# kpreid/all-is-cubes

Measured on NVIDIA H100. Metric: Mrays/s, higher is better.
Workload: dtype f64 geometry / f32 colour

## Files before the change

### all-is-cubes_b200/csrc/aicb200.cu

```cuda
#include <algorithm>
#include <array>
#include <cmath>
#include <cstdio>
#include <cstdlib>
#include <cstring>
#include <initializer_list>
#include <mutex>
#include <string>
#include <unordered_map>
#include <vector>

#include <cuda_runtime.h>

#include "brick_room.h"
#include "internal.h"

using namespace aicb;

static thread_local std::string g_last_error = "";

aicb_status aicb_fail(aicb_status st, const std::string &msg) {
    g_last_error = msg;
    return st;
}
// ... 117 lines not shown
    const uint32_t pal = pal_off + pal_base;
    float palf;
    std::memcpy(&palf, &pal, 4);
    return make_float4(e.x, e.y, palf, 0.0f);
}

static aicb_status flatten_block(const aicb_block_desc &b, BlockRec &r, uint8_t &kind, std::vector<uint16_t> &bricks,
                                 std::vector<float4> &palette, std::vector<float2> &pal_tab) {
    std::memset(&r, 0, sizeof r);
    const uint32_t res = b.resolution;
    if (res == 0 || (res & (res - 1)) || res > 128) return fail(AICB_ERR_INVALID, "block resolution must be 1..128, power of 2");
    auto push_voxel = [&](const aicb_voxel &v) {
        palette.push_back(make_float4(v.rgba[0], v.rgba[1], v.rgba[2], v.rgba[3]));
        palette.push_back(make_float4(v.emission[0], v.emission[1], v.emission[2], 0.0f));
        pal_tab.push_back(surface_entry(v.rgba[3]));
    };
    bool single = false;
    aicb_voxel sv = AIR_VOXEL;
    if (b.indices == nullptr) {
        single = true;
        if (b.n_palette) {
            if (!b.palette) return fail(AICB_ERR_INVALID, "palette is NULL");
            sv = b.palette[0];
        }
    } else {
        const uint64_t nvox = (uint64_t)b.voxel_bounds.size[0] * b.voxel_bounds.size[1] * b.voxel_bounds.size[2];
        if (nvox != b.n_indices) return fail(AICB_ERR_INVALID, "n_indices does not match voxel_bounds");
        for (int a = 0; a < 3; a++) {
            int64_t lo = b.voxel_bounds.lower[a], hi = lo + (int64_t)b.voxel_bounds.size[a];
            if (lo < 0 || hi > (int64_t)res) return fail(AICB_ERR_INVALID, "voxel_bounds must lie within [0, resolution)^3");
        }
        if (!b.palette && b.n_palette) return fail(AICB_ERR_INVALID, "palette is NULL");
        for (size_t k = 0; k < b.n_indices; k++)
            if (b.indices[k] >= b.n_palette) return fail(AICB_ERR_INVALID, "voxel index out of palette range");
        if (res == 1) {
            single = true;
            sv = (nvox == 1 && b.voxel_bounds.lower[0] == 0 && b.voxel_bounds.lower[1] == 0 && b.voxel_bounds.lower[2] == 0)
                     ? b.palette[b.indices[0]]
                     : AIR_VOXEL;
        }
    }
    if (b.is_air) {
        kind = KIND_INVISIBLE;
        r.kind_res = KIND_INVISIBLE | (1u << 8);
    } else if (single) {
        kind = voxel_invisible(sv) ? KIND_INVISIBLE : KIND_SINGLE;
        r.kind_res = kind | (1u << 8);
        r.pal_off = (uint32_t)(palette.size() / 2);
        r.vsize[0] = r.vsize[1] = r.vsize[2] = 1;
        push_voxel(sv);
    } else {
        if (b.n_palette > 32768) return fail(AICB_ERR_UNSUPPORTED, "block palettes above 32768 entries are not supported");
        kind = KIND_RECURSIVE;
        r.kind_res = KIND_RECURSIVE | (res << 8);
        for (int a = 0; a < 3; a++) {
            r.vlo[a] = (int16_t)b.voxel_bounds.lower[a];
            r.vsize[a] = (uint16_t)b.voxel_bounds.size[a];
        }
        if (bricks.size() + b.n_indices > 0xffffffffull) return fail(AICB_ERR_INVALID, "brick pool exceeds 2^32 voxels");
        r.brick_off = (uint32_t)bricks.size();
        r.pal_off = (uint32_t)(palette.size() / 2);
        for (size_t k = 0; k < b.n_indices; k++) {
            uint16_t v = b.indices[k];
            bricks.push_back((uint16_t)(v | (voxel_invisible(b.palette[v]) ? 0x8000u : 0u)));
        }
        for (size_t k = 0; k < b.n_palette; k++) push_voxel(b.palette[k]);
    }
    return AICB_OK;
}

typedef void (*kernel_fn)(const TraceParams, uint32_t);

template <bool V, bool W, bool AUX>
static kernel_fn kernel_of() {
    return trace_kernel<V, W, AUX>;
}

static kernel_fn select_kernel(bool volumetric, bool wide, bool aux) {
#define PICK(V, W, A) if (volumetric == V && wide == W && aux == A) return kernel_of<V, W, A>();
    PICK(false, false, false) PICK(false, false, true) PICK(false, true, false) PICK(false, true, true)
    PICK(true, false, false) PICK(true, false, true) PICK(true, true, false) PICK(true, true, true)
#undef PICK
    return nullptr;
}

template <typename... KArgs, typename... Args>
static cudaError_t launch_after(bool overlap, void (*kern)(KArgs...), unsigned grid, unsigned block, cudaStream_t st, Args... args) {
    cudaLaunchConfig_t cfg;
    std::memset(&cfg, 0, sizeof cfg);
    cfg.gridDim = dim3(grid, 1, 1);
    cfg.blockDim = dim3(block, 1, 1);
    cfg.dynamicSmemBytes = 0;
    cfg.stream = st;
    cudaLaunchAttribute attr[1];
    attr[0].id = cudaLaunchAttributeProgrammaticStreamSerialization;
    attr[0].val.programmaticStreamSerializationAllowed = 1;
    cfg.attrs = attr;
    cfg.numAttrs = overlap ? 1 : 0;
    return cudaLaunchKernelEx(&cfg, kern, args...);
}

struct CubeDelta {
    uint32_t idx, cell, light, has_light;
};

static __global__ void scatter_cubes_kernel(const CubeDelta *ops, uint32_t n, uint32_t wide, void *cells, uint32_t *light) {
    const uint32_t i = blockIdx.x * blockDim.x + threadIdx.x;
    if (i >= n) return;
    const CubeDelta op = ops[i];
    if (wide) ((uint32_t *)cells)[op.idx] = op.cell; else ((uint16_t *)cells)[op.idx] = (uint16_t)op.cell;
    if (op.has_light) light[op.idx] = op.light;
}

static __device__ __forceinline__ uint32_t widened_cell(uint32_t w) { return (w & 0x3fffu) | ((w >> 14) << 16); }

static __global__ void __launch_bounds__(256) widen_cells_kernel(const uint16_t *__restrict__ in, uint32_t *__restrict__ out,
                                                                 size_t n) {
    const size_t stride = (size_t)gridDim.x * blockDim.x, first = (size_t)blockIdx.x * blockDim.x + threadIdx.x;
    const size_t n8 = n / 8;
    for (size_t i = first; i < n8; i += stride) {
        const uint4 v = __ldcs(reinterpret_cast<const uint4 *>(in) + i);
        __stcs(reinterpret_cast<uint4 *>(out) + 2 * i,
               make_uint4(widened_cell(v.x & 0xffffu), widened_cell(v.x >> 16), widened_cell(v.y & 0xffffu),
                          widened_cell(v.y >> 16)));
        __stcs(reinterpret_cast<uint4 *>(out) + 2 * i + 1,
               make_uint4(widened_cell(v.z & 0xffffu), widened_cell(v.z >> 16), widened_cell(v.w & 0xffffu),
                          widened_cell(v.w >> 16)));
    }
    for (size_t i = n8 * 8 + first; i < n; i += stride) out[i] = widened_cell(in[i]);
}

static __global__ void __launch_bounds__(256) fill_cells_kernel(uint16_t *__restrict__ cells, size_t n, uint32_t word) {
    const size_t stride = (size_t)gridDim.x * blockDim.x, first = (size_t)blockIdx.x * blockDim.x + threadIdx.x;
    const uint32_t pair = word | word << 16;
    const size_t n8 = n / 8;
    for (size_t i = first; i < n8; i += stride) __stcs(reinterpret_cast<uint4 *>(cells) + i, make_uint4(pair, pair, pair, pair));
    for (size_t i = n8 * 8 + first; i < n; i += stride) cells[i] = (uint16_t)word;
}

struct PoolSegment {
    uint64_t src, dst, bytes;
};

static __global__ void __launch_bounds__(256) compact_pool_kernel(const uint8_t *__restrict__ src, uint8_t *__restrict__ dst,
                                                                  const PoolSegment *__restrict__ segs, uint32_t n_segs) {
    for (uint32_t k = blockIdx.x; k < n_segs; k += gridDim.x) {
        const PoolSegment g = segs[k];
        const uint64_t shift = g.src - g.dst;
        const uint64_t c0 = (g.dst + 15) / 16, c1 = (g.dst + g.bytes) / 16;
        const uint32_t s = (uint32_t)(shift & 15), b = (s & 3) * 8;
        for (uint64_t c = c0 + threadIdx.x; c < c1; c += blockDim.x) {
            const uint4 *p = reinterpret_cast<const uint4 *>(src + ((c * 16 + shift) & ~15ull));
            const uint4 lo = p[0];
            uint4 out = lo;
            if (s) {
                const uint4 hi = p[1];
                const uint32_t w[8] = {lo.x, lo.y, lo.z, lo.w, hi.x, hi.y, hi.z, hi.w};
#define FS(i) __funnelshift_r(w[i], w[(i) + 1], b)
                switch (s >> 2) {
                    case 0: out = make_uint4(FS(0), FS(1), FS(2), FS(3)); break;
                    case 1: out = make_uint4(FS(1), FS(2), FS(3), FS(4)); break;
                    case 2: out = make_uint4(FS(2), FS(3), FS(4), FS(5)); break;
                    default: out = make_uint4(FS(3), FS(4), FS(5), FS(6)); break;
                }
#undef FS
            }
// ... 120 lines not shown
    P.task_counter = ctx->d_tile_counter;
    P.refill_threshold = REFILL_THRESHOLD;
    P.tail_divisor = TAIL_DIVISOR;
    P.event_threshold = EVENT_THRESHOLD;

    sc->pending = true;
    sc->pending_pixels = pixels;
    sc->pending_rays = pixels * (P.antialias ? 4 : 1);
    sc->pending_out_bytes_per_pixel =
        P.target.out_srgb8 ? 4 : (tgt == TGT_TEX ? 12 : (tgt == TGT_TERM ? 24 : (P.target.out_rgba16f ? 8 : 16)));

    P.n_samples = P.antialias ? 4 : 1;
    const bool fused = (opt->lighting_display == AICB_LIGHT_NONE || opt->lighting_display == AICB_LIGHT_FLAT) &&
                       !ctx->deep_frames;
    const uint64_t total_tasks = (uint64_t)P.n_tasks * P.n_samples;
    uint64_t CHUNK = (uint64_t)4 << 20;
    {
        const uint64_t per_task = sizeof(RayRecordA) + sizeof(RayRecordB) + sizeof(TaskOut) + 4 * N_BINS +
                                  (uint64_t)ctx->hits_per_task * (sizeof(HitRecord) + (fused ? 0 : sizeof(ShadedHit)));
        uint64_t fit = ((uint64_t)8 << 30) / per_task;
        if (fit < (1u << 17)) fit = 1u << 17;
        if (fit < CHUNK) CHUNK = fit & ~(uint64_t)127;
    }
    const uint64_t chunk_cap = total_tasks < CHUNK ? total_tasks : CHUNK;
    uint64_t cap = chunk_cap * ctx->hits_per_task;
    if (cap < (1u << 16)) cap = 1u << 16;
    if (cap > 0xfffffff0ull) cap = 0xfffffff0ull;
    cap &= ~(uint64_t)(HIT_CHUNK - 1);
    P.hit_capacity = (uint32_t)cap;
    TRY(ctx->primary.size(chunk_cap, P.hit_capacity, !fused));
    ctx->primary.bind(P, chunk_cap, !fused);
    P.ray_counter = ctx->d_tile_counter + 2;
    sc->pending_fused = fused;
    P.hit_counter = ctx->d_tile_counter + 1;
    P.bin_count = ctx->d_tile_counter + 4;
    P.bin_stride = (uint32_t)chunk_cap;
    P.overflow_flag = (unsigned int *)(P.counters + 7);
    if (stream != ctx->stream.get()) CU(cudaStreamWaitEvent(stream, ctx->ev_delta.get(), 0));
    if (ctx->frame_in_flight && ctx->last_stream != stream) CU(cudaStreamWaitEvent(stream, ctx->ev1.get(), 0));
    ctx->frame_in_flight = true;
    ctx->last_stream = stream;
    ctx->last_scene = sc;
    CU(cudaMemsetAsync(P.counters, 0, 8 * sizeof(unsigned long long) + 2 * (4 + N_BINS) * sizeof(unsigned int), stream));
    CU(cudaEventRecord(ctx->ev0.get(), stream));
    if (total_tasks > 0) {
        const bool volumetric = opt->transparency == AICB_TRANSPARENCY_VOLUMETRIC;
        const int lc = opt->lighting_display == AICB_LIGHT_NONE ? LC_NONE
                       : (opt->lighting_display == AICB_LIGHT_FLAT ? LC_FLAT
                          : (opt->lighting_display == AICB_LIGHT_BOUNCE ? LC_BOUNCE : LC_INTERP));
        TraceParams Q;
        const bool bounce = lc == LC_BOUNCE;
        if (bounce) {
            TRY(ctx->secondary.size(chunk_cap, P.hit_capacity, true));
            TRY(ctx->d_bounce.ensure(chunk_cap * 104 + 256));
            char *b = ctx->d_bounce.get<char>();
            P.bounce_mode = BOUNCE_PRIMARY;
            P.bounce_samples = opt->bounce_samples;
            P.bounce_rays = (double *)b;
            P.bounce_rng = (unsigned long long *)(b + chunk_cap * 48);
            P.bounce_sum = (float4 *)(b + chunk_cap * 80);
            P.bounce_req = (uint32_t *)(b + chunk_cap * 96);
            P.ray_index = (uint32_t *)(b + chunk_cap * 100);
            Q = P;
            Q.ray_index = nullptr;
            Q.bounce_mode = BOUNCE_SECONDARY;
            Q.rays = P.bounce_rays;
            Q.tiles_y = 1;
            Q.shard_count = 1; Q.shard_index = 0; Q.strip_rows = 1;
            Q.antialias = 0;
            Q.n_samples = 1;
            Q.task_base = 0;
            Q.lighting = AICB_LIGHT_FLAT;
            Q.include_sky = 1;
            Q.exposure = 1.0f;
            Q.out_full_frame = 0;
            Q.target = {};
            ctx->secondary.bind(Q, chunk_cap, true);
            Q.task_counter = ctx->d_tile_counter + (4 + N_BINS);
            Q.hit_counter = Q.task_counter + 1;
            Q.ray_counter = Q.task_counter + 2;
            Q.bin_count = Q.task_counter + 4;
            Q.debug_warp_times = nullptr;
        }
        kernel_fn k = select_kernel(volumetric, sc->ds.wide_cells != 0, out.aux);
        int blocks_per_sm = 0;
        CU(cudaOccupancyMaxActiveBlocksPerMultiprocessor(&blocks_per_sm, k, WARPS_PER_BLOCK * 32, 0));
        if (blocks_per_sm < 1) blocks_per_sm = 1;
        for (uint64_t base = 0; base < total_tasks; base += CHUNK) {
            const uint32_t n = (uint32_t)(total_tasks - base < CHUNK ? total_tasks - base : CHUNK);
            P.task_base = (uint32_t)base;
            const bool first = base == 0;
            if (!first) CU(cudaMemsetAsync(ctx->d_tile_counter, 0, (4 + N_BINS) * sizeof(unsigned int), stream));
            const bool prof = ctx->profile_kernels && first;
            const bool stage = first && ctx->stage_timing;
            if (stage) cudaEventRecord(ctx->ev_k[0].get(), stream);
            gen_kernel<<<(n + 127) / 128, 128, 0, stream>>>(P, n);
            if (stage) cudaEventRecord(ctx->ev_k[1].get(), stream);
            uint64_t want = ((uint64_t)n + WARPS_PER_BLOCK * 32 - 1) / (WARPS_PER_BLOCK * 32);
            uint64_t grid = (uint64_t)ctx->num_sms * blocks_per_sm;
            if (grid > want) grid = want;
            if (prof) {
                TRY(ctx->d_debug.ensure(4 * 8 * (size_t)ctx->num_sms * 64 * WARPS_PER_BLOCK));
                P.debug_warp_times = ctx->d_debug.get<unsigned long long>();
                ctx->debug_warps = (uint32_t)grid * WARPS_PER_BLOCK;
            }
            const bool overlap = !stage && !prof && !bounce;
            CU(launch_after(overlap, k, (unsigned)grid, WARPS_PER_BLOCK * 32, stream, P, n));
            P.debug_warp_times = nullptr;
            if (stage) cudaEventRecord(ctx->ev_k[2].get(), stream);
            if (fused) {
                const unsigned rb = (n + 127) / 128;
                CU(launch_after(overlap, resolve_for(lc, tgt), rb, 128, stream, P, n));
                if (stage) cudaEventRecord(ctx->ev_k[3].get(), stream);
            } else if (!bounce) {
                switch (lc) {
                    case LC_NONE: CU(launch_after(overlap, shade_kernel<LC_NONE>, ctx->num_sms * SHADE_BLOCKS_PER_SM, 128, stream, P)); break;
                    case LC_FLAT: CU(launch_after(overlap, shade_kernel<LC_FLAT>, ctx->num_sms * SHADE_BLOCKS_PER_SM, 128, stream, P)); break;
                    default: CU(launch_after(overlap, shade_kernel<LC_INTERP>, ctx->num_sms * SHADE_BLOCKS_PER_SM, 128, stream, P)); break;
                }
                if (stage) cudaEventRecord(ctx->ev_k[3].get(), stream);
                const uint32_t n_pixels = n / P.n_samples;
                CU(launch_after(overlap, encode_for(tgt), (n_pixels + 127) / 128, 128, stream, P, n));
                if (stage) cudaEventRecord(ctx->ev_k[4].get(), stream);
            } else {
                shade_kernel<LC_BOUNCE><<<ctx->num_sms * SHADE_BLOCKS_PER_SM, 128, 0, stream>>>(P);
                const unsigned tb = (n + 127) / 128;
                bounce_select_kernel<<<tb, 128, 0, stream>>>(P, n);
                Q.n_rays = n;
                Q.n_tasks = n;
                Q.tiles_x = (n + 31) / 32;
                for (uint32_t pass = 0; pass < P.bounce_samples; pass++) {
                    Q.bounce_pass = pass;
                    CU(cudaMemsetAsync(Q.task_counter, 0, (4 + N_BINS) * sizeof(unsigned int), stream));
                    bounce_gen_kernel<<<tb, 128, 0, stream>>>(P, n);
                    gen_kernel<<<tb, 128, 0, stream>>>(Q, n);
                    k<<<(unsigned)grid, WARPS_PER_BLOCK * 32, 0, stream>>>(Q, n);
                    shade_kernel<LC_FLAT><<<ctx->num_sms * SHADE_BLOCKS_PER_SM, 128, 0, stream>>>(Q);
                    encode_kernel<TGT_FRAME><<<tb, 128, 0, stream>>>(Q, n);
                }
                bounce_resolve_kernel<<<tb, 128, 0, stream>>>(P, n);
                if (stage) cudaEventRecord(ctx->ev_k[3].get(), stream);
                const uint32_t n_pixels = n / P.n_samples;
                encode_for(tgt)<<<(n_pixels + 127) / 128, 128, 0, stream>>>(P, n);
                if (stage) cudaEventRecord(ctx->ev_k[4].get(), stream);
            }
        }
        CU(cudaGetLastError());
    }
    CU(cudaEventRecord(ctx->ev1.get(), stream));
    return AICB_OK;
}

static aicb_status finish(aicb_scene *sc, aicb_render_info *info) {
    aicb_ctx *ctx = sc->ctx;
    if (ctx->last_scene != sc)
        return fail(AICB_ERR_BUSY, "the context's last frame belongs to another scene (one frame per context is tracked)");
    CU(cudaEventSynchronize(ctx->ev1.get()));
    ctx->frame_in_flight = false;
    unsigned long long c[8];
    CU(cudaMemcpy(c, ctx->d_counters.get(), sizeof c, cudaMemcpyDeviceToHost));
    sc->pending = false;
    if (ctx->profile_kernels && sc->pending_rays) {
        float t[4] = {0, 0, 0, 0};
        for (int i = 0; i < (sc->pending_fused ? 3 : 4); i++) cudaEventElapsedTime(&t[i], ctx->ev_k[i].get(), ctx->ev_k[i + 1].get());
        if (ctx->d_debug && ctx->debug_warps) {
            std::vector<unsigned long long> w(4 * (size_t)ctx->debug_warps);
            cudaMemcpy(w.data(), ctx->d_debug.get(), w.size() * 8, cudaMemcpyDeviceToHost);
            unsigned long long t0 = ~0ull, t1 = 0, passes = 0, rays = 0;
            for (uint32_t i = 0; i < ctx->debug_warps; i++) { t0 = std::min(t0, w[4 * i]); t1 = std::max(t1, w[4 * i + 1]); passes += w[4 * i + 2]; rays += w[4 * i + 3]; }
            std::vector<double> ends;
// ... 1279 lines not shown
```

### all-is-cubes_b200/csrc/internal.h

```cpp
#pragma once
#include <memory>
#include <mutex>
#include <string>
#include <utility>
#include <vector>

#include <cuda_runtime.h>

#include "trace_kernel.cuh"

aicb_status aicb_fail(aicb_status st, const std::string &msg);
aicb_status aicb_cuda_fail(cudaError_t e, const char *what);
#define CU(call)                                                   \
    do {                                                           \
        cudaError_t e__ = (call);                                  \
        if (e__ != cudaSuccess) return aicb_cuda_fail(e__, #call); \
    } while (0)
#define TRY(call)                                  \
    do {                                           \
        aicb_status st__ = (call);                 \
        if (st__ != AICB_OK) return st__;          \
    } while (0)

struct DeviceMemory {
// ... 55 lines not shown
};
using DeviceBuffer = Buffer<DeviceMemory>;
using PinnedBuffer = Buffer<PinnedMemory>;

struct EventDestroy {
    void operator()(cudaEvent_t e) const { cudaEventDestroy(e); }
};
struct StreamDestroy {
    void operator()(cudaStream_t s) const { cudaStreamDestroy(s); }
};
using Event = std::unique_ptr<CUevent_st, EventDestroy>;
using Stream = std::unique_ptr<CUstream_st, StreamDestroy>;

inline aicb_status create_event(Event &e, unsigned int flags) {
    cudaEvent_t raw = nullptr;
    CU(cudaEventCreateWithFlags(&raw, flags));
    e.reset(raw);
    return AICB_OK;
}

inline uint32_t cell_word(uint32_t id, uint8_t kind, bool wide) { return id | ((uint32_t)kind << (wide ? 16 : 14)); }

struct ChunkStreams {
    DeviceBuffer rays, task_out, hits, shaded, bin_list;

    aicb_status size(uint64_t chunk_cap, uint32_t hit_capacity, bool shade) {
        TRY(rays.ensure(chunk_cap * (sizeof(aicb::RayRecordA) + sizeof(aicb::RayRecordB)) + 16));
        TRY(task_out.ensure(chunk_cap * sizeof(aicb::TaskOut) + 16));
        TRY(hits.ensure((size_t)hit_capacity * sizeof(aicb::HitRecord) + 64));
        if (shade) TRY(shaded.ensure((size_t)hit_capacity * sizeof(aicb::ShadedHit) + 64));
        return bin_list.ensure((size_t)aicb::N_BINS * chunk_cap * 4 + 64);
    }
    void bind(aicb::TraceParams &P, uint64_t chunk_cap, bool shade) const {
        P.rays_a = rays.get<aicb::RayRecordA>();
        P.rays_b = (aicb::RayRecordB *)(rays.get<char>() + chunk_cap * sizeof(aicb::RayRecordA));
        P.task_out = task_out.get<aicb::TaskOut>();
        P.hits = hits.get<aicb::HitRecord>();
        P.shaded = shade ? shaded.get<aicb::ShadedHit>() : nullptr;
        P.bin_list = bin_list.get<uint32_t>();
    }
    void release_hits() {
        hits.reset();
        shaded.reset();
    }
};

struct LightChart {
    DeviceBuffer pre, chains, node_rel, euler, term_scratch;
    uint32_t nodes = 0, n_chains = 0, n_euler = 0, walk_blocks = 0;
};

struct LightState {
    struct Own {
        DeviceBuffer sky_term;
        DeviceBuffer overflow;
        DeviceBuffer overflow_count;
    } own;
    struct Shared {
        DeviceBuffer pending;
        DeviceBuffer tile_max;
        DeviceBuffer list, new_light, diff;
        DeviceBuffer counters;
        DeviceBuffer changes;
        DeviceBuffer dirty, push_targets;
    } shared;

    aicb_status ensure(aicb_scene *s, size_t replica, size_t n_replicas, const std::vector<float4> *terms);

    uint32_t *changed() const { return own.overflow.get<uint32_t>(); }
    uint32_t *chunk_sums() const { return shared.diff.get<uint32_t>(); }
    uint32_t *taken_indices() const { return shared.list.get<uint32_t>(); }
    uint32_t *taken_texels() const { return shared.new_light.get<uint32_t>(); }
};

struct aicb_ctx {
    int device = 0;
    int num_sms = 0;
    Stream stream;
    Event ev0, ev1;
    Event ev_light[2];
    Event ev_join;
    Event ev_k[5];
    bool profile_kernels = false;
    bool stage_timing = true;
    PinnedBuffer h_delta;
    DeviceBuffer d_delta;
    Event ev_delta;
    DeviceBuffer d_debug;
    uint32_t debug_warps = 0;
    DeviceBuffer d_counters;
    unsigned int *d_tile_counter = nullptr;
    DeviceBuffer d_lut;
    DeviceBuffer d_out, d_aux;
    ChunkStreams primary, secondary;
    DeviceBuffer d_bounce;
    uint32_t hits_per_task = 8;
    uint32_t shallow_frames = 0;
    bool deep_frames = false;
    PinnedBuffer h_stage;
    bool frame_in_flight = false;
    cudaStream_t last_stream = nullptr;
    struct aicb_scene *last_scene = nullptr;
    DeviceBuffer d_task_aux;
    DeviceBuffer d_task_depth;
    DeviceBuffer d_task_text;
    LightChart light_chart;
    std::mutex mu;
};

struct BlockTable {
    struct Extent {
        uint32_t brick_off, n_bricks;
        uint32_t pal_off, n_pal;
    };

    DeviceBuffer blocks;
    DeviceBuffer blk_tab;
    DeviceBuffer light;
    DeviceBuffer bricks;
    DeviceBuffer palette;
    DeviceBuffer pal_tab;
    std::vector<uint8_t> kind;
    std::vector<uint32_t> light_flags;
    std::vector<Extent> extent;
    size_t n_bricks = 0, n_palette = 0;
    size_t dead_bricks = 0, dead_pal = 0;

    size_t block_count() const { return kind.size(); }
    size_t bytes() const {
        return block_count() * (sizeof(aicb::BlockRec) + sizeof(float4) + sizeof(LightBlockDev)) + n_bricks * 2 +
               n_palette * sizeof(float4) + n_palette / 2 * sizeof(float2);
    }
    void bind(aicb::DeviceScene &ds) const {
        ds.blocks = blocks.get<aicb::BlockRec>();
        ds.blk_tab = blk_tab.get<float4>();
        ds.bricks = bricks.get<uint16_t>();
        ds.palette = palette.get<float4>();
        ds.pal_tab = pal_tab.get<float2>();
    }
};

struct aicb_scene {
    aicb_ctx *ctx = nullptr;
    aicb::DeviceScene ds{};
    size_t volume = 0;
    uint64_t device_bytes = 0;
    DeviceBuffer d_cells;
    DeviceBuffer d_light;
    BlockTable blocks;
    bool pending = false;
    uint64_t pending_rays = 0;
    uint64_t pending_pixels = 0;
    uint32_t pending_out_bytes_per_pixel = 0;
    bool pending_fused = false;
    std::vector<uint16_t> h_ids;
    LightState light;
    uint32_t light_max_distance = 0;
    uint64_t light_stats[4] = {0, 0, 0, 0};
};

struct Outputs {
    aicb::TargetParams target{};
    int kind = aicb::TGT_FRAME;
    bool full_frame = false;
    bool aux = false;
    const double *rays = nullptr;
// ... 88 lines not shown
```

### all-is-cubes_b200/csrc/trace_kernel.cuh

```cuda
#pragma once
#include <cstdint>
#include <type_traits>
#include <cuda_runtime.h>

#include "../../include/aicb200.h"

#ifdef __CUDACC__
#include <cuda_fp16.h>
#endif

struct LightBlockDev {
    float face_color[7][4];
    float emission[3];
    uint32_t flags;
};
static_assert(sizeof(LightBlockDev) == 128, "LightBlockDev must be 128 bytes");

namespace aicb {

constexpr uint32_t KIND_SINGLE = 0;
constexpr uint32_t KIND_RECURSIVE = 1;
constexpr uint32_t KIND_INVISIBLE = 2;

struct BlockRec {
// ... 710 lines not shown
        lv.base = 0;
        Caster c;
        c.tmx = c.tmy = c.tmz = c.last_t = 0.0;
        c.rx = c.ry = c.rz = 0;
        c.face = 0;
        c.idx = 0;
        bool valid;
        running = caster_begin(c, r, o[0], o[1], o[2], lv, &valid);
        rec.ox = r.ox; rec.oy = r.oy; rec.oz = r.oz; rec.dx = r.dx; rec.dy = r.dy; rec.dz = r.dz;
        rb.tdx = r.tdx; rb.tdy = r.tdy; rb.tdz = r.tdz;
        rb.half_over_len = r.half_over_len;
        rb.tmx = c.tmx; rb.tmy = c.tmy; rb.tmz = c.tmz; rb.last_t = c.last_t;
        rb.rx = c.rx; rb.ry = c.ry; rb.rz = c.rz;
        rb.task = i;
        rec.flags = ((uint32_t)c.face & 7u) | (running ? 8u : 0u) | (valid ? 16u : 0u) | 32u | ((uint32_t)(r.sx + 1) << 6) |
                    ((uint32_t)(r.sy + 1) << 8) | ((uint32_t)(r.sz + 1) << 10) | (octant << 12);
        if (running) {
            const float lo3[3] = {(float)lv.lox, (float)lv.loy, (float)lv.loz};
            const float n3[3] = {(float)lv.nx, (float)lv.ny, (float)lv.nz};
            float tn = 0.0f, tf = 3.0e38f, l1 = 0.0f;
#pragma unroll
            for (int a = 0; a < 3; a++) {
                const float da = (float)d[a], oa = (float)o[a];
                if (da != 0.0f) {
                    const float t0 = (lo3[a] - oa) / da, t1 = (lo3[a] + n3[a] - oa) / da;
                    tn = fmaxf(tn, fminf(t0, t1));
                    tf = fminf(tf, fmaxf(t0, t1));
                    l1 += fabsf(da);
                }
            }
            const float crossings = fmaxf(tf - tn, 0.0f) * l1;
            const float frac = crossings / (n3[0] + n3[1] + n3[2]);
            int q = (int)(frac * (float)N_BINS);
            q = q < 0 ? 0 : (q > N_BINS - 1 ? N_BINS - 1 : q);
            bin = N_BINS - 1 - q;
        }
    }
    }
    const unsigned listed = __ballot_sync(0xffffffffu, running);
    if (running) {
        const int lane = (int)(threadIdx.x & 31);
        const unsigned below = listed & ((1u << lane) - 1u);
        uint32_t rbase = 0;
        if (below == 0) rbase = atomicAdd(P.ray_counter, (unsigned)__popc(listed));
        rbase = __shfl_sync(listed, rbase, __ffs(listed) - 1);
        const uint32_t r = rbase + __popc(below);
        const unsigned peers = __match_any_sync(listed, bin);
        const int leader = __ffs(peers) - 1;
        uint32_t base = 0;
        if (lane == leader) base = atomicAdd(P.bin_count + bin, (unsigned)__popc(peers));
        base = __shfl_sync(peers, base, leader);
        const uint32_t slot = base + __popc(peers & ((1u << lane) - 1u));
        P.bin_list[(size_t)bin * P.bin_stride + slot] = r;
        if (P.ray_index) P.ray_index[i] = r;
        const uint4 *src = reinterpret_cast<const uint4 *>(&rec);
        uint4 *dst = reinterpret_cast<uint4 *>(P.rays_a + r);
#pragma unroll
        for (int k = 0; k < 4; k++) st_stream(dst + k, src[k]);
        src = reinterpret_cast<const uint4 *>(&rb);
        dst = reinterpret_cast<uint4 *>(P.rays_b + r);
#pragma unroll
        for (int k = 0; k < 5; k++) st_stream(dst + k, src[k]);
    } else if (in_range) {
        TaskOut o;
        o.first_hit = 0xffffffffu;
        o.steps = 0;
        o.flags = octant;
        o.n_hits = 0;
        *reinterpret_cast<uint4 *>(P.task_out + i) = *reinterpret_cast<const uint4 *>(&o);
    }
}

template <bool VOLUMETRIC, bool WIDE, bool AUX>
__global__ void __launch_bounds__(WARPS_PER_BLOCK * 32, AUX ? 1 : MIN_BLOCKS_PER_SM)
trace_kernel(const __grid_constant__ TraceParams P, uint32_t n_chunk_tasks) {
    grid_dependency_sync();
    const DeviceScene &S = P.scene;
    const int lane = threadIdx.x & 31;
    constexpr float F_NEG_INF = -__builtin_huge_valf();
    constexpr int COUNTER_STATIC = 0x3fffffff;

    unsigned long long n_outer = 0, n_inner = 0, n_blocks = 0;

    __shared__ double sh_d[13][WARPS_PER_BLOCK * 32];
    __shared__ uint32_t sh_w[13][WARPS_PER_BLOCK * 32];
    __shared__ uint4 sh_stash[VOLUMETRIC ? 3 : 1][WARPS_PER_BLOCK * 32];
    const int tid = threadIdx.x;
#define COLD_D(k) sh_d[k][tid]
#define COLD_W(k) sh_w[k][tid]
#define STASH(k) sh_stash[k][tid]
    __shared__ double sh_t_scale[WARPS_PER_BLOCK * 32];
    __shared__ uint32_t sh_hits[3][WARPS_PER_BLOCK * 32];
    __shared__ unsigned long long sh_dbg[3][WARPS_PER_BLOCK * 32];
    unsigned long long &dbg_t0 = sh_dbg[0][tid], &dbg_passes = sh_dbg[1][tid], &dbg_rays = sh_dbg[2][tid];
    dbg_t0 = dbg_passes = dbg_rays = 0;
    if (P.debug_warp_times) {
        unsigned long long t0;
        asm volatile("mov.u64 %0, %%globaltimer;" : "=l"(t0));
        dbg_t0 = t0;
    }

    __shared__ uint32_t s_bin_start[N_BINS + 1];
    if (threadIdx.x == 0) {
        uint32_t acc = 0;
        for (int b = 0; b < N_BINS; b++) { s_bin_start[b] = acc; acc += P.bin_count[b]; }
        s_bin_start[N_BINS] = acc;
    }
    __syncthreads();
    const uint32_t n_listed = s_bin_start[N_BINS];
    (void)n_chunk_tasks;

    int st = ST_IDLE;
    double tmx = 0.0, tmy = 0.0, tmz = 0.0, last_t = 0.0;
    double tdx = 0.0, tdy = 0.0, tdz = 0.0;
    double &t_scale = sh_t_scale[tid];
    t_scale = 1.0;
    uint32_t idx = 0;
    int stx = 0, sty = 0, stz = 0;
    int cx = 0, cy = 0, cz = 0;
    int fcx = 0, fcy = 0, fcz = 0;
    int face = 0;
    uint32_t sbits = 0;
    bool valid = false, inner = false, need_advance = false, have_pending = false;
    float L = 0.0f;
    uint32_t steps = 0, step_limit = 1000u;
    uint32_t &n_hits = sh_hits[0][tid];
    uint32_t &chunk_base = sh_hits[1][tid], &chunk_used = sh_hits[2][tid];
    n_hits = 0;
    chunk_base = HIT_NONE;
    chunk_used = HIT_CHUNK;
    uint32_t ev_word = 0;
    AuxState<AUX> aux{};
    bool list_exhausted = false;

    auto bound_factor = [&](float p) {
        L = (p < -8.5f) ? F_NEG_INF : L + (p + 1e-4f);
        step_limit = (L < -8.0f) ? 0u : 1000u;
    };

    auto advance = [&]() -> bool {
        const bool xy = tmx < tmy, xz = tmx < tmz, yz = tmy < tmz;
        const bool ax = xy & xz;
        const bool ay = !xy & yz;
        const bool axy = ax | ay;
        const double tm = ax ? tmx : (ay ? tmy : tmz);
        const double td = ax ? tdx : (ay ? tdy : tdz);
        const double nt = tm + td;
        last_t = tm;
        tmx = ax ? nt : tmx;
        tmy = ay ? nt : tmy;
        tmz = axy ? tmz : nt;
        idx += (uint32_t)(ax ? stx : (ay ? sty : stz));
        face = ax ? fcx : (ay ? fcy : fcz);
        cx -= ax ? 1 : 0;
        cy -= ay ? 1 : 0;
        cz -= axy ? 0 : 1;
        return (cx | cy | cz) < 0;
    };

    auto advance_branchy = [&]() -> bool {
        if ((tmx < tmy) & (tmx < tmz)) {
            last_t = tmx; tmx = tmx + tdx; idx += (uint32_t)stx; face = fcx; cx -= 1;
            return cx < 0;
        } else if (tmy < tmz) {
            last_t = tmy; tmy = tmy + tdy; idx += (uint32_t)sty; face = fcy; cy -= 1;
            return cy < 0;
        } else {
            last_t = tmz; tmz = tmz + tdz; idx += (uint32_t)stz; face = fcz; cz -= 1;
            return cz < 0;
        }
    };

    auto take_slot = [&]() -> uint32_t {
        if (chunk_used == HIT_CHUNK) {
            const uint32_t nb = atomicAdd(P.hit_counter, HIT_CHUNK);
            if (nb + HIT_CHUNK > P.hit_capacity) {
                *P.overflow_flag = 1u;
                chunk_base = HIT_NONE;
            } else {
                if (chunk_base != HIT_NONE && n_hits != 0) P.hits[chunk_base + HIT_CHUNK - 1].next = nb;
                chunk_base = nb;
            }
            chunk_used = 0;
        }
        uint32_t slot = HIT_NONE;
        if (chunk_base != HIT_NONE) {
            slot = chunk_base + chunk_used;
            chunk_used++;
            if (n_hits == 0) COLD_W(7) = slot;
            n_hits++;
        }
        return slot;
    };

    auto store_record = [&](uint32_t slot, uint4 q0, uint4 q1, uint4 q2, float thickness) {
        uint4 *dst = reinterpret_cast<uint4 *>(P.hits + slot);
        st_stream(dst, q0);
        st_stream(dst + 1, q1);
        st_stream(dst + 2, q2);
        st_stream(dst + 3, make_uint4(__float_as_uint(thickness), steps, COLD_W(6), HIT_NONE));
    };

    auto emit_surface = [&](uint32_t word) {
        uint32_t entry;
        float2 te;
        if (inner) {
            entry = COLD_W(9) + word;
            te = __ldg(S.pal_tab + entry);
        } else {
            const float4 t4 = __ldg(S.blk_tab + word);
            te = make_float2(t4.x, t4.y);
            entry = __float_as_uint(t4.z);
        }
        const uint4 q0 = make_uint4((uint32_t)__double2loint(tmx), (uint32_t)__double2hiint(tmx),
                                    (uint32_t)__double2loint(tmy), (uint32_t)__double2hiint(tmy));
        const uint4 q1 = make_uint4((uint32_t)__double2loint(tmz), (uint32_t)__double2hiint(tmz),
                                    (uint32_t)__double2loint(last_t), (uint32_t)__double2hiint(last_t));
        const uint4 q2 = make_uint4(entry, inner ? COLD_W(0) : idx, idx,
                                    (uint32_t)face | (inner ? (8u | (COLD_W(10) << 4)) : 0u));
        if constexpr (VOLUMETRIC) {
            STASH(0) = q0;
            STASH(1) = q1;
            STASH(2) = q2;
            COLD_W(11) = __float_as_uint(te.y);
            COLD_D(12) = last_t * t_scale;
            have_pending = true;
        } else {
            const uint32_t slot = take_slot();
            if (slot != HIT_NONE) store_record(slot, q0, q1, q2, 0.0f);
            if (P.transparency == AICB_TRANSPARENCY_THRESHOLD) {
                if (te.x > P.threshold) L = F_NEG_INF;
            } else {
                bound_factor(te.y);
            }
        }
    };

    auto step = [&](auto lean) {
        bool left = false;
        if (need_advance) {
            if (!valid) {
                st = inner ? ST_POP : ST_DONE;
                return;
            }
            if constexpr (decltype(lean)::value) left = advance_branchy(); else left = advance();
        }
        need_advance = true;
        uint32_t w = 0;
        if (!left) {
            if constexpr (WIDE) {
                if (!inner) {
                    const uint32_t cell = __ldg((const uint32_t *)S.cells + idx);
                    w = (cell & 0x3fffu) | ((cell >> 2) & 0xc000u);
                    ev_word = cell & 0xffffu;
                } else {
                    w = __ldg(S.bricks + idx);
                }
            } else {
                w = __ldg((inner ? S.bricks : (const uint16_t *)S.cells) + idx);
            }
            if constexpr (AUX) { if (inner) aux.n_inner++; else aux.n_outer++; }
        }
        steps += 1;
        if (steps > step_limit) { st = ST_DONE; return; }
        if constexpr (VOLUMETRIC) {
            if (have_pending) {
                const float th = fmaxf((float)((last_t * t_scale - COLD_D(12)) * COLD_D(7)), 0.0f);
                const float pend_l2a = __uint_as_float(COLD_W(11));
                const uint32_t slot = take_slot();
                if (slot != HIT_NONE) store_record(slot, STASH(0), STASH(1), STASH(2), th);
                bound_factor(pend_l2a == F_NEG_INF ? F_NEG_INF : th * pend_l2a);
                have_pending = false;
            }
        }
        if (left) {
            st = inner ? ST_POP : ST_DONE;
            return;
        }
        if (w & 0x8000u) return;
        if (!inner && (w & 0x4000u)) {
            if constexpr (VOLUMETRIC) {
                steps += 1;
                if (steps > step_limit) { st = ST_DONE; return; }
            }
            if constexpr (!WIDE) ev_word = w & 0x3fffu;
            st = ST_ENTER;
            return;
        }
        if constexpr (WIDE) emit_surface(inner ? w : ev_word);
        else emit_surface(inner ? w : (w & 0x3fffu));
    };

    for (;;) {
        dbg_passes++;
        if (st == ST_DONE) {
            dbg_rays++;
            TaskOut o;
            o.first_hit = COLD_W(7);
            o.steps = steps;
            o.flags = COLD_W(8);
            o.n_hits = n_hits;
            *reinterpret_cast<uint4 *>(P.task_out + COLD_W(12)) = *reinterpret_cast<const uint4 *>(&o);
            if constexpr (AUX) { n_outer += aux.n_outer; n_inner += aux.n_inner; n_blocks += aux.n_blocks; }
            st = ST_IDLE;
        }
        {
            const unsigned idle = __ballot_sync(0xffffffffu, st == ST_IDLE);
            if (idle && !list_exhausted) {
                const int n = __popc(idle);
                uint32_t base = 0;
                const int leader = __ffs(idle) - 1;
                if (lane == leader) base = atomicAdd(P.task_counter, (unsigned)n);
                base = __shfl_sync(0xffffffffu, base, leader);
                if (st == ST_IDLE) {
                    const uint32_t k = base + __popc(idle & ((1u << lane) - 1u));
                    if (k >= n_listed) {
                        st = ST_EXHAUSTED;
                    } else {
                        int b = 0;
                        while (k >= s_bin_start[b + 1]) b++;
                        const uint32_t ri = __ldg(P.bin_list + (size_t)b * P.bin_stride + (k - s_bin_start[b]));
                        RayRecordA rec;
                        RayRecordB rb;
                        {
                            const uint4 *src = reinterpret_cast<const uint4 *>(P.rays_a + ri);
                            uint4 *dst = reinterpret_cast<uint4 *>(&rec);
#pragma unroll
                            for (int q = 0; q < 4; q++) dst[q] = ld_stream(src + q);
                            src = reinterpret_cast<const uint4 *>(P.rays_b + ri);
                            dst = reinterpret_cast<uint4 *>(&rb);
#pragma unroll
                            for (int q = 0; q < 5; q++) dst[q] = __ldcs(src + q);
                        }
                        const uint32_t task = rb.task;
                        COLD_W(6) = ri;
                        COLD_W(12) = task;
                        COLD_D(0) = rec.ox; COLD_D(1) = rec.oy; COLD_D(2) = rec.oz;
                        COLD_D(3) = rec.dx; COLD_D(4) = rec.dy; COLD_D(5) = rec.dz;
                        COLD_D(6) = rb.half_over_len;
                        COLD_D(7) = rec.t_to_abs;
                        COLD_W(7) = HIT_NONE;
                        COLD_W(8) = (rec.flags >> 12) & 7u;
                        tdx = rb.tdx; tdy = rb.tdy; tdz = rb.tdz;
                        tmx = rb.tmx; tmy = rb.tmy; tmz = rb.tmz; last_t = rb.last_t;
                        sbits = (rec.flags >> 6) & 0x3fu;
                        const int sx = (int)(sbits & 3u) - 1, sy = (int)((sbits >> 2) & 3u) - 1, sz = (int)((sbits >> 4) & 3u) - 1;
                        fcx = sx > 0 ? AICB_FACE_NX : AICB_FACE_PX;
                        fcy = sy > 0 ? AICB_FACE_NY : AICB_FACE_PY;
                        fcz = sz > 0 ? AICB_FACE_NZ : AICB_FACE_PZ;
                        stx = sx * (S.size[1] * S.size[2]); sty = sy * S.size[2]; stz = sz;
                        cx = sx > 0 ? S.size[0] - 1 - rb.rx : (sx < 0 ? rb.rx : COUNTER_STATIC);
                        cy = sy > 0 ? S.size[1] - 1 - rb.ry : (sy < 0 ? rb.ry : COUNTER_STATIC);
                        cz = sz > 0 ? S.size[2] - 1 - rb.rz : (sz < 0 ? rb.rz : COUNTER_STATIC);
                        idx = (uint32_t)((rb.rx * S.size[1] + rb.ry) * S.size[2] + rb.rz);
                        face = (int)(rec.flags & 7u);
                        valid = (rec.flags & 16u) != 0;
                        L = 0.0f;
                        step_limit = 1000u;
                        if (P.target.in_accum) {
                            const float t0 = __ldg(&P.target.in_accum[P.task_base + task].w);
                            L = (t0 > 0.0f) ? __log2f(t0) + 1e-3f : F_NEG_INF;
                            step_limit = (L < -8.0f) ? 0u : 1000u;
                        }
                        steps = 0;
                        n_hits = 0;
                        have_pending = false;
                        inner = false;
                        t_scale = 1.0;
                        need_advance = false;
                        if constexpr (AUX) aux.n_outer = aux.n_inner = aux.n_blocks = 0;
                        st = ST_MARCH;
                    }
                }
                if (__any_sync(0xffffffffu, st == ST_EXHAUSTED)) list_exhausted = true;
            }
            if (__all_sync(0xffffffffu, st == ST_EXHAUSTED || st == ST_IDLE)) break;
        }
        if (st == ST_ENTER) {
            if constexpr (AUX) aux.n_blocks++;
            const uint4 *bp = reinterpret_cast<const uint4 *>(S.blocks + ev_word);
            const uint4 b0 = __ldg(bp);
            const uint4 b1 = __ldg(bp + 1);
            const int bres = (int)(b0.x >> 8);
            Level in;
            in.lox = (int16_t)(b0.y & 0xffff); in.loy = (int16_t)(b0.y >> 16); in.loz = (int16_t)(b0.z & 0xffff);
            in.nx = (int)(b0.z >> 16); in.ny = (int)(b0.w & 0xffff); in.nz = (int)(b0.w >> 16);
            in.base = b1.x;
            const double fres = (double)bres;
            const uint32_t nyz = (uint32_t)S.size[1] * (uint32_t)S.size[2];
            const uint32_t qx = idx / nyz, rem = idx - qx * nyz;
            const uint32_t qy = rem / (uint32_t)S.size[2], qz = rem - qy * (uint32_t)S.size[2];
            const int ccx = (int)qx + S.lo[0], ccy = (int)qy + S.lo[1], ccz = (int)qz + S.lo[2];
            Ray rr;
            rr.ox = COLD_D(0); rr.oy = COLD_D(1); rr.oz = COLD_D(2);
            rr.dx = COLD_D(3); rr.dy = COLD_D(4); rr.dz = COLD_D(5);
            rr.tdx = tdx; rr.tdy = tdy; rr.tdz = tdz;
            rr.half_over_len = COLD_D(6);
            rr.sx = (int)(sbits & 3u) - 1; rr.sy = (int)((sbits >> 2) & 3u) - 1; rr.sz = (int)((sbits >> 4) & 3u) - 1;
            Caster ic;
            bool ivalid;
            if (caster_begin(ic, rr, (rr.ox - (double)ccx) * fres, (rr.oy - (double)ccy) * fres, (rr.oz - (double)ccz) * fres, in,
                             &ivalid)) {
                COLD_D(8) = tmx; COLD_D(9) = tmy; COLD_D(10) = tmz; COLD_D(11) = last_t;
                COLD_W(0) = idx; COLD_W(1) = (uint32_t)cx; COLD_W(2) = (uint32_t)cy; COLD_W(3) = (uint32_t)cz;
                COLD_W(4) = (uint32_t)face; COLD_W(5) = valid ? 1u : 0u;
                COLD_W(9) = b1.y;
                COLD_W(10) = (uint32_t)(31 - __clz(bres));
                tmx = ic.tmx; tmy = ic.tmy; tmz = ic.tmz; last_t = ic.last_t;
                idx = ic.idx;
                face = ic.face;
                valid = ivalid;
                cx = rr.sx > 0 ? in.nx - 1 - ic.rx : (rr.sx < 0 ? ic.rx : COUNTER_STATIC);
                cy = rr.sy > 0 ? in.ny - 1 - ic.ry : (rr.sy < 0 ? ic.ry : COUNTER_STATIC);
                cz = rr.sz > 0 ? in.nz - 1 - ic.rz : (rr.sz < 0 ? ic.rz : COUNTER_STATIC);
                stx = rr.sx * (in.ny * in.nz); sty = rr.sy * in.nz; stz = rr.sz;
                inner = true;
                t_scale = recip_pow2(bres);
                need_advance = false;
            }
            st = ST_MARCH;
        }
        if (st == ST_POP) {
            tmx = COLD_D(8); tmy = COLD_D(9); tmz = COLD_D(10); last_t = COLD_D(11);
            idx = COLD_W(0); cx = (int)COLD_W(1); cy = (int)COLD_W(2); cz = (int)COLD_W(3);
            face = (int)COLD_W(4);
            valid = COLD_W(5) != 0;
            const int sx = (int)(sbits & 3u) - 1, sy = (int)((sbits >> 2) & 3u) - 1, sz = (int)((sbits >> 4) & 3u) - 1;
            stx = sx * (S.size[1] * S.size[2]); sty = sy * S.size[2]; stz = sz;
            inner = false;
            t_scale = 1.0;
            need_advance = true;
            st = ST_MARCH;
        }
        {
            const int n_off = __popc(__ballot_sync(0xffffffffu, st == ST_EXHAUSTED || (list_exhausted && st == ST_IDLE)));
            int thr = (int)P.event_threshold;
            if (list_exhausted) {
                const int tail_div = (int)P.tail_divisor;
                thr = (32 - n_off) / (tail_div > 0 ? tail_div : 2);
                thr = thr < 1 ? 1 : (thr > (int)P.event_threshold ? (int)P.event_threshold : thr);
            }
            const unsigned live = __ballot_sync(0xffffffffu, st == ST_MARCH);
            if (list_exhausted && __popc(live) <= (int)P.refill_threshold) {
                if (st == ST_MARCH) {
                    do { step(std::true_type{}); } while (st == ST_MARCH);
                }
            } else {
                for (;;) {
                    const unsigned marching = __ballot_sync(0xffffffffu, st == ST_MARCH);
                    if (!marching) break;
                    if (32 - __popc(marching) - n_off >= thr) break;
                    if (st == ST_MARCH) step(std::false_type{});
                }
            }
        }
        __syncwarp();
    }

    if (P.debug_warp_times) {
        unsigned long long t1;
        asm volatile("mov.u64 %0, %%globaltimer;" : "=l"(t1));
        unsigned long long rays = dbg_rays;
        for (int off = 16; off > 0; off >>= 1) rays += __shfl_down_sync(0xffffffffu, rays, off);
        if (lane == 0) {
            unsigned long long *d = P.debug_warp_times + 4 * (size_t)(blockIdx.x * WARPS_PER_BLOCK + (threadIdx.x >> 5));
            d[0] = dbg_t0; d[1] = t1; d[2] = dbg_passes; d[3] = rays;
        }
    }
    if (chunk_base != HIT_NONE)
        for (uint32_t j = chunk_used; j < HIT_CHUNK; j++) P.hits[chunk_base + j].thickness = -2.0f;

    if constexpr (AUX) {
#pragma unroll
        for (int off = 16; off > 0; off >>= 1) {
            n_outer += __shfl_down_sync(0xffffffffu, n_outer, off);
            n_inner += __shfl_down_sync(0xffffffffu, n_inner, off);
            n_blocks += __shfl_down_sync(0xffffffffu, n_blocks, off);
        }
        if (lane == 0) {
            atomicAdd(P.counters + 1, n_outer);
            atomicAdd(P.counters + 2, n_inner);
            atomicAdd(P.counters + 5, n_blocks);
        }
    }
#undef COLD_D
#undef COLD_W
#undef STASH
}

struct HitGeom {
    int cube[3];
    int voxel[3];
    int res;
    int face;
    uint32_t pal;
};
AICB_DEV void decode_hit(const DeviceScene &S, const HitRecord &h, HitGeom &g) {
    const uint32_t nz = (uint32_t)S.size[2], nyz = (uint32_t)S.size[1] * nz;
    const uint32_t qx = h.cell / nyz, rem = h.cell - qx * nyz;
    const uint32_t qy = rem / nz, qz = rem - qy * nz;
    g.cube[0] = (int)qx + S.lo[0]; g.cube[1] = (int)qy + S.lo[1]; g.cube[2] = (int)qz + S.lo[2];
    g.face = (int)(h.flags & 7u);
    if (h.flags & 8u) {
        const uint32_t id = S.wide_cells ? (__ldg((const uint32_t *)S.cells + h.cell) & 0xffffu)
                                         : ((uint32_t)__ldg((const uint16_t *)S.cells + h.cell) & 0x3fffu);
        const uint4 *bp = reinterpret_cast<const uint4 *>(S.blocks + id);
        const uint4 b0 = __ldg(bp);
        const uint32_t brick_off = __ldg(bp + 1).x;
        const uint32_t vny = b0.w & 0xffffu, vnz = b0.w >> 16;
        const uint32_t local = h.vidx - brick_off;
        const uint32_t vx = local / (vny * vnz), vrem = local - vx * (vny * vnz);
        const uint32_t vy = vrem / vnz, vz = vrem - vy * vnz;
        g.voxel[0] = (int)vx + (int)(int16_t)(b0.y & 0xffff);
        g.voxel[1] = (int)vy + (int)(int16_t)(b0.y >> 16);
        g.voxel[2] = (int)vz + (int)(int16_t)(b0.z & 0xffff);
        g.res = 1 << ((h.flags >> 4) & 15u);
    } else {
        g.voxel[0] = g.voxel[1] = g.voxel[2] = 0;
        g.res = 1;
    }
    g.pal = h.pal;
}

template <int LC>
AICB_DEV ShadedHit shade_hit(const TraceParams &P, const float *s_lut, const uint32_t i, const float *illum_override,
                             unsigned long long &texels) {
    const DeviceScene &S = P.scene;
    const bool volumetric = P.transparency == AICB_TRANSPARENCY_VOLUMETRIC;
    const bool have_fog = (P.fog != AICB_FOG_NONE) && P.include_sky;
    const float fog_blend = (P.fog == AICB_FOG_ABRUPT) ? 1.0f : (P.fog == AICB_FOG_COMPROMISE ? 0.5f : 0.0f);
    HitRecord h;
    {
        const uint4 *src = reinterpret_cast<const uint4 *>(P.hits + i);
        uint4 *dst = reinterpret_cast<uint4 *>(&h);
#pragma unroll
        for (int k = 0; k < 4; k++) dst[k] = ld_stream(src + k);
    }
    const RayRecordA *rp = P.rays_a + h.task;
    const float4 col = __ldg(S.palette + 2 * (size_t)h.pal);
    const float4 emi = __ldg(S.palette + 2 * (size_t)h.pal + 1);
    const uint2 rmeta = __ldg(reinterpret_cast<const uint2 *>(&rp->t_to_view));
    const uint32_t rflags = rmeta.y;
    Ray rr;
    rr.ox = rr.oy = rr.oz = rr.dx = rr.dy = rr.dz = 0.0;
    if constexpr (LC == LC_INTERP) {
        const double2 *q = reinterpret_cast<const double2 *>(rp);
        const double2 q0 = __ldg(q), q1 = __ldg(q + 1), q2 = __ldg(q + 2);
        rr.ox = q0.x; rr.oy = q0.y; rr.oz = q1.x; rr.dx = q1.y; rr.dy = q2.x; rr.dz = q2.y;
    }
// ... 680 lines not shown
```

Baseline: 2676.

## Shrink trace kernel shared memory and pick a fitting carve-out step

Cuts per-thread shared-memory state in the trace kernel: ray origin and direction are no longer cached in shared memory but re-read from global when a recursive block is entered, and per-thread debug counters become per-warp. A host helper picks the smallest shared-memory carve-out step that still holds the occupancy-limited number of resident blocks and caches that choice per kernel variant. The intent is to free shared memory, leaving more for L1, at the cost of extra global loads on each recursive-block entry.

```diff
diff --git a/all-is-cubes_b200/csrc/aicb200.cu b/all-is-cubes_b200/csrc/aicb200.cu
--- a/all-is-cubes_b200/csrc/aicb200.cu
+++ b/all-is-cubes_b200/csrc/aicb200.cu
@@ -223,6 +223,42 @@
     PICK(true, false, false) PICK(true, false, true) PICK(true, true, false) PICK(true, true, true)
 #undef PICK
     return nullptr;
+}
+
+#ifndef AICB_MARCH_CARVEOUT_STEPS_UP
+#define AICB_MARCH_CARVEOUT_STEPS_UP 0
+#endif
+
+static aicb_status march_kernel(aicb_ctx *ctx, bool volumetric, bool wide, bool aux, kernel_fn *kernel, int *blocks_per_sm) {
+    static const int STEPS_KB[] = {0, 8, 16, 32, 64, 100, 132, 164, 196, 228};
+    constexpr int N_STEPS = (int)(sizeof STEPS_KB / sizeof STEPS_KB[0]);
+    kernel_fn k = select_kernel(volumetric, wide, aux);
+    *kernel = k;
+    int &cached = ctx->march_blocks[(volumetric ? 4 : 0) | (wide ? 2 : 0) | (aux ? 1 : 0)];
+    if (cached == 0) {
+        CU(cudaFuncSetAttribute(k, cudaFuncAttributePreferredSharedMemoryCarveout, cudaSharedmemCarveoutMaxShared));
+        int blocks = 0;
+        CU(cudaOccupancyMaxActiveBlocksPerMultiprocessor(&blocks, k, WARPS_PER_BLOCK * 32, 0));
+        if (blocks < 1) return fail(AICB_ERR_CUDA, "the marching kernel does not fit an SM");
+        cudaFuncAttributes fa;
+        CU(cudaFuncGetAttributes(&fa, k));
+        int reserved = 0, sm_max = 0;
+        CU(cudaDeviceGetAttribute(&reserved, cudaDevAttrReservedSharedMemoryPerBlock, ctx->device));
+        CU(cudaDeviceGetAttribute(&sm_max, cudaDevAttrMaxSharedMemoryPerMultiprocessor, ctx->device));
+        const size_t need = (size_t)blocks * (fa.sharedSizeBytes + (size_t)reserved);
+        int step = 0;
+        while (step < N_STEPS - 1 && (size_t)STEPS_KB[step] * 1024 < need) step++;
+        step = std::min(step + AICB_MARCH_CARVEOUT_STEPS_UP, N_STEPS - 1);
+        for (int fit = 0; fit < blocks; step++) {
+            if (step >= N_STEPS) return fail(AICB_ERR_CUDA, "no shared-memory carve-out holds the marching kernel's resident blocks");
+            const int percent = (int)((size_t)STEPS_KB[step] * 1024 * 100 / (size_t)sm_max);
+            CU(cudaFuncSetAttribute(k, cudaFuncAttributePreferredSharedMemoryCarveout, percent));
+            CU(cudaOccupancyMaxActiveBlocksPerMultiprocessor(&fit, k, WARPS_PER_BLOCK * 32, 0));
+        }
+        cached = blocks;
+    }
+    *blocks_per_sm = cached;
+    return AICB_OK;
 }
 
 template <typename... KArgs, typename... Args>
@@ -509,10 +545,9 @@
             Q.bin_count = Q.task_counter + 4;
             Q.debug_warp_times = nullptr;
         }
-        kernel_fn k = select_kernel(volumetric, sc->ds.wide_cells != 0, out.aux);
+        kernel_fn k = nullptr;
         int blocks_per_sm = 0;
-        CU(cudaOccupancyMaxActiveBlocksPerMultiprocessor(&blocks_per_sm, k, WARPS_PER_BLOCK * 32, 0));
-        if (blocks_per_sm < 1) blocks_per_sm = 1;
+        TRY(march_kernel(ctx, volumetric, sc->ds.wide_cells != 0, out.aux, &k, &blocks_per_sm));
         for (uint64_t base = 0; base < total_tasks; base += CHUNK) {
             const uint32_t n = (uint32_t)(total_tasks - base < CHUNK ? total_tasks - base : CHUNK);
             P.task_base = (uint32_t)base;
diff --git a/all-is-cubes_b200/csrc/internal.h b/all-is-cubes_b200/csrc/internal.h
--- a/all-is-cubes_b200/csrc/internal.h
+++ b/all-is-cubes_b200/csrc/internal.h
@@ -161,6 +161,7 @@
     Event ev_join;
     Event ev_k[5];
     bool profile_kernels = false;
+    int march_blocks[8] = {};
     bool stage_timing = true;
     PinnedBuffer h_delta;
     DeviceBuffer d_delta;
diff --git a/all-is-cubes_b200/csrc/trace_kernel.cuh b/all-is-cubes_b200/csrc/trace_kernel.cuh
--- a/all-is-cubes_b200/csrc/trace_kernel.cuh
+++ b/all-is-cubes_b200/csrc/trace_kernel.cuh
@@ -816,7 +816,7 @@
 
     unsigned long long n_outer = 0, n_inner = 0, n_blocks = 0;
 
-    __shared__ double sh_d[13][WARPS_PER_BLOCK * 32];
+    __shared__ double sh_d[VOLUMETRIC ? 7 : 6][WARPS_PER_BLOCK * 32];
     __shared__ uint32_t sh_w[13][WARPS_PER_BLOCK * 32];
     __shared__ uint4 sh_stash[VOLUMETRIC ? 3 : 1][WARPS_PER_BLOCK * 32];
     const int tid = threadIdx.x;
@@ -825,16 +825,19 @@
 #define STASH(k) sh_stash[k][tid]
     __shared__ double sh_t_scale[WARPS_PER_BLOCK * 32];
     __shared__ uint32_t sh_hits[3][WARPS_PER_BLOCK * 32];
-    __shared__ unsigned long long sh_dbg[3][WARPS_PER_BLOCK * 32];
-    unsigned long long &dbg_t0 = sh_dbg[0][tid], &dbg_passes = sh_dbg[1][tid], &dbg_rays = sh_dbg[2][tid];
-    dbg_t0 = dbg_passes = dbg_rays = 0;
-    if (P.debug_warp_times) {
+    __shared__ unsigned long long sh_dbg[3][WARPS_PER_BLOCK];
+    const int warp = threadIdx.x >> 5;
+    if (P.debug_warp_times && lane == 0) {
         unsigned long long t0;
         asm volatile("mov.u64 %0, %%globaltimer;" : "=l"(t0));
-        dbg_t0 = t0;
+        sh_dbg[0][warp] = t0;
+        sh_dbg[1][warp] = sh_dbg[2][warp] = 0;
     }
 
     __shared__ uint32_t s_bin_start[N_BINS + 1];
+    static_assert(MIN_BLOCKS_PER_SM * (sizeof sh_d + sizeof sh_w + sizeof sh_stash + sizeof sh_t_scale + sizeof sh_hits +
+                                       sizeof sh_dbg + sizeof s_bin_start + 1024) <= (VOLUMETRIC ? 132u : 100u) * 1024u,
+                  "trace_kernel's shared memory crosses a carve-out step: 132 KB (Volumetric) or 100 KB for 5 blocks");
     if (threadIdx.x == 0) {
         uint32_t acc = 0;
         for (int b = 0; b < N_BINS; b++) { s_bin_start[b] = acc; acc += P.bin_count[b]; }
@@ -957,7 +960,7 @@
             STASH(1) = q1;
             STASH(2) = q2;
             COLD_W(11) = __float_as_uint(te.y);
-            COLD_D(12) = last_t * t_scale;
+            COLD_D(6) = last_t * t_scale;
             have_pending = true;
         } else {
             const uint32_t slot = take_slot();
@@ -999,7 +1002,7 @@
         if (steps > step_limit) { st = ST_DONE; return; }
         if constexpr (VOLUMETRIC) {
             if (have_pending) {
-                const float th = fmaxf((float)((last_t * t_scale - COLD_D(12)) * COLD_D(7)), 0.0f);
+                const float th = fmaxf((float)((last_t * t_scale - COLD_D(6)) * COLD_D(1)), 0.0f);
                 const float pend_l2a = __uint_as_float(COLD_W(11));
                 const uint32_t slot = take_slot();
                 if (slot != HIT_NONE) store_record(slot, STASH(0), STASH(1), STASH(2), th);
@@ -1026,9 +1029,11 @@
     };
 
     for (;;) {
-        dbg_passes++;
+        if (P.debug_warp_times) {
+            const int done = __popc(__ballot_sync(0xffffffffu, st == ST_DONE));
+            if (lane == 0) { sh_dbg[1][warp]++; sh_dbg[2][warp] += (unsigned)done; }
+        }
         if (st == ST_DONE) {
-            dbg_rays++;
             TaskOut o;
             o.first_hit = COLD_W(7);
             o.steps = steps;
@@ -1054,30 +1059,25 @@
                         int b = 0;
                         while (k >= s_bin_start[b + 1]) b++;
                         const uint32_t ri = __ldg(P.bin_list + (size_t)b * P.bin_stride + (k - s_bin_start[b]));
-                        RayRecordA rec;
+                        const uint4 ra = ld_stream(reinterpret_cast<const uint4 *>(P.rays_a + ri) + 3);
+                        const uint32_t rflags = ra.y;
                         RayRecordB rb;
                         {
-                            const uint4 *src = reinterpret_cast<const uint4 *>(P.rays_a + ri);
-                            uint4 *dst = reinterpret_cast<uint4 *>(&rec);
-#pragma unroll
-                            for (int q = 0; q < 4; q++) dst[q] = ld_stream(src + q);
-                            src = reinterpret_cast<const uint4 *>(P.rays_b + ri);
-                            dst = reinterpret_cast<uint4 *>(&rb);
+                            const uint4 *src = reinterpret_cast<const uint4 *>(P.rays_b + ri);
+                            uint4 *dst = reinterpret_cast<uint4 *>(&rb);
 #pragma unroll
                             for (int q = 0; q < 5; q++) dst[q] = __ldcs(src + q);
                         }
                         const uint32_t task = rb.task;
                         COLD_W(6) = ri;
                         COLD_W(12) = task;
-                        COLD_D(0) = rec.ox; COLD_D(1) = rec.oy; COLD_D(2) = rec.oz;
-                        COLD_D(3) = rec.dx; COLD_D(4) = rec.dy; COLD_D(5) = rec.dz;
-                        COLD_D(6) = rb.half_over_len;
-                        COLD_D(7) = rec.t_to_abs;
+                        COLD_D(0) = rb.half_over_len;
+                        COLD_D(1) = __hiloint2double((int)ra.w, (int)ra.z);
                         COLD_W(7) = HIT_NONE;
-                        COLD_W(8) = (rec.flags >> 12) & 7u;
+                        COLD_W(8) = (rflags >> 12) & 7u;
                         tdx = rb.tdx; tdy = rb.tdy; tdz = rb.tdz;
                         tmx = rb.tmx; tmy = rb.tmy; tmz = rb.tmz; last_t = rb.last_t;
-                        sbits = (rec.flags >> 6) & 0x3fu;
+                        sbits = (rflags >> 6) & 0x3fu;
                         const int sx = (int)(sbits & 3u) - 1, sy = (int)((sbits >> 2) & 3u) - 1, sz = (int)((sbits >> 4) & 3u) - 1;
                         fcx = sx > 0 ? AICB_FACE_NX : AICB_FACE_PX;
                         fcy = sy > 0 ? AICB_FACE_NY : AICB_FACE_PY;
@@ -1087,8 +1087,8 @@
                         cy = sy > 0 ? S.size[1] - 1 - rb.ry : (sy < 0 ? rb.ry : COUNTER_STATIC);
                         cz = sz > 0 ? S.size[2] - 1 - rb.rz : (sz < 0 ? rb.rz : COUNTER_STATIC);
                         idx = (uint32_t)((rb.rx * S.size[1] + rb.ry) * S.size[2] + rb.rz);
-                        face = (int)(rec.flags & 7u);
-                        valid = (rec.flags & 16u) != 0;
+                        face = (int)(rflags & 7u);
+                        valid = (rflags & 16u) != 0;
                         L = 0.0f;
                         step_limit = 1000u;
                         if (P.target.in_accum) {
@@ -1115,6 +1115,8 @@
             const uint4 *bp = reinterpret_cast<const uint4 *>(S.blocks + ev_word);
             const uint4 b0 = __ldg(bp);
             const uint4 b1 = __ldg(bp + 1);
+            const double2 *rp = reinterpret_cast<const double2 *>(P.rays_a + COLD_W(6));
+            const double2 r0 = __ldg(rp), r1 = __ldg(rp + 1), r2 = __ldg(rp + 2);
             const int bres = (int)(b0.x >> 8);
             Level in;
             in.lox = (int16_t)(b0.y & 0xffff); in.loy = (int16_t)(b0.y >> 16); in.loz = (int16_t)(b0.z & 0xffff);
@@ -1126,16 +1128,16 @@
             const uint32_t qy = rem / (uint32_t)S.size[2], qz = rem - qy * (uint32_t)S.size[2];
             const int ccx = (int)qx + S.lo[0], ccy = (int)qy + S.lo[1], ccz = (int)qz + S.lo[2];
             Ray rr;
-            rr.ox = COLD_D(0); rr.oy = COLD_D(1); rr.oz = COLD_D(2);
-            rr.dx = COLD_D(3); rr.dy = COLD_D(4); rr.dz = COLD_D(5);
+            rr.ox = r0.x; rr.oy = r0.y; rr.oz = r1.x;
+            rr.dx = r1.y; rr.dy = r2.x; rr.dz = r2.y;
             rr.tdx = tdx; rr.tdy = tdy; rr.tdz = tdz;
-            rr.half_over_len = COLD_D(6);
+            rr.half_over_len = COLD_D(0);
             rr.sx = (int)(sbits & 3u) - 1; rr.sy = (int)((sbits >> 2) & 3u) - 1; rr.sz = (int)((sbits >> 4) & 3u) - 1;
             Caster ic;
             bool ivalid;
             if (caster_begin(ic, rr, (rr.ox - (double)ccx) * fres, (rr.oy - (double)ccy) * fres, (rr.oz - (double)ccz) * fres, in,
                              &ivalid)) {
-                COLD_D(8) = tmx; COLD_D(9) = tmy; COLD_D(10) = tmz; COLD_D(11) = last_t;
+                COLD_D(2) = tmx; COLD_D(3) = tmy; COLD_D(4) = tmz; COLD_D(5) = last_t;
                 COLD_W(0) = idx; COLD_W(1) = (uint32_t)cx; COLD_W(2) = (uint32_t)cy; COLD_W(3) = (uint32_t)cz;
                 COLD_W(4) = (uint32_t)face; COLD_W(5) = valid ? 1u : 0u;
                 COLD_W(9) = b1.y;
@@ -1155,7 +1157,7 @@
             st = ST_MARCH;
         }
         if (st == ST_POP) {
-            tmx = COLD_D(8); tmy = COLD_D(9); tmz = COLD_D(10); last_t = COLD_D(11);
+            tmx = COLD_D(2); tmy = COLD_D(3); tmz = COLD_D(4); last_t = COLD_D(5);
             idx = COLD_W(0); cx = (int)COLD_W(1); cy = (int)COLD_W(2); cz = (int)COLD_W(3);
             face = (int)COLD_W(4);
             valid = COLD_W(5) != 0;
@@ -1194,11 +1196,9 @@
     if (P.debug_warp_times) {
         unsigned long long t1;
         asm volatile("mov.u64 %0, %%globaltimer;" : "=l"(t1));
-        unsigned long long rays = dbg_rays;
-        for (int off = 16; off > 0; off >>= 1) rays += __shfl_down_sync(0xffffffffu, rays, off);
         if (lane == 0) {
-            unsigned long long *d = P.debug_warp_times + 4 * (size_t)(blockIdx.x * WARPS_PER_BLOCK + (threadIdx.x >> 5));
-            d[0] = dbg_t0; d[1] = t1; d[2] = dbg_passes; d[3] = rays;
+            unsigned long long *d = P.debug_warp_times + 4 * (size_t)(blockIdx.x * WARPS_PER_BLOCK + warp);
+            d[0] = sh_dbg[0][warp]; d[1] = t1; d[2] = sh_dbg[1][warp]; d[3] = sh_dbg[2][warp];
         }
     }
     if (chunk_base != HIT_NONE)
```

Result: no change. 2688 (median of 6 runs) (+0.4%).
